# facebookresearch/iSDF

Measured on AMD Instinct MI355X. Metric: train-steps/sec: device-synchronised Trainer.step() on 27k-point ray batches, timed as metrics.start_timing / end_timing bracket it (SURVEY 8d); whole job.  SDF L1 vs GT: sdf_l1_vs_gt, higher is better.
Workload: dtype f16 MFMA operands (compensated forward: hi+lo operands past the cat layer), f32 accumulate; second-order sweeps and dW operands fp16; 1 GPU; replicaCAD.json defaults: 5 keyframes x 200 rays x 27 samples = 27000 points per rank-step, 680x1200 synthetic room depth, 6x256 Softplus MLP + 255-wide icosahedron PE (460033 params), eik+normal loss, bounds=ray, AdamW; stream=680x1200, scaling_mode=weak: every rank draws the full 5 x 200 rays, parallelism=single GPU

## Files before the change

isdf_amd/csrc/capi.hip:

```cpp
#include <cstdio>
#include "isdf_common.h"
#include "chain_params.h"
#include "launchers.h"

using namespace isdf;

namespace isdf { thread_local int g_isdf_last_hip_error = 0; }

extern "C" {

int isdf_abi_version(void) { return ISDF_ABI_VERSION; }

static thread_local int g_isdf_last_collective_error = 0;

const char* isdf_error_string(int code) {
  switch (code) {
    case ISDF_OK: return "ok";
    case ISDF_EINVAL: return "invalid argument";
    case ISDF_EUNSUPPORTED: return "unsupported configuration (the tile kernels take hidden_feature_size <= 512 (zero-padded to 256 / 512), n_freqs = n_embed_funcs+1 in 1..12, any hidden_layers_block up to 7; bounds_method ray|pc)";
    case ISDF_EWORKSPACE: return "workspace too small";
    case ISDF_EHIP: {
      static thread_local char buf[160];
      snprintf(buf, sizeof(buf), "HIP runtime error: %s", g_isdf_last_hip_error ? hipGetErrorString((hipError_t)g_isdf_last_hip_error) : "(no launch status recorded)");
      return buf;
    }
    case ISDF_ECOLLECTIVE: {
      static thread_local char buf[96];
      snprintf(buf, sizeof(buf), "the collective library refused the all-reduce (ncclResult_t %d)", g_isdf_last_collective_error);
      return buf;
    }
  }
  return "unknown error";
}

int isdf_check_net(const isdf_net_cfg* net) {
  NetLayout l; int rc = make_layout(net, &l);
  if (rc) return rc;
  return layout_supported(l) ? ISDF_OK : ISDF_EUNSUPPORTED;
}

int64_t isdf_param_count(const isdf_net_cfg* net) {
  NetLayout l; int rc = make_layout(net, &l);
  return rc ? rc : l.n_params;
}

int64_t isdf_shadow_bytes(const isdf_net_cfg* net) {
  NetLayout l; int rc = make_layout(net, &l);
  return rc ? rc : l.shadowElems * 2;
}

int64_t isdf_workspace_bytes(const isdf_net_cfg* net, int64_t max_points, int32_t train) {
  NetLayout l; int rc = make_layout(net, &l);
  if (rc) return rc;
  if (max_points < 0) return ISDF_EINVAL;
  WorkspaceLayout w; make_workspace(l, max_points, max_points, train != 0, &w);
  return w.totalBytes;
}

int64_t isdf_reduce_floats(const isdf_net_cfg* net, int32_t n_frames) {
  NetLayout l; int rc = make_layout(net, &l);
  if (rc) return rc;
  return reduce_layout(l, n_frames).total;
}

int64_t isdf_reduce_split_floats(const isdf_net_cfg* net) {
  NetLayout l; int rc = make_layout(net, &l);
  if (rc) return rc;
  return l.offW[l.cat];
}

int isdf_pack_weights(const isdf_net_cfg* net, const float* params, void* shadow, void* stream) {
  isdf_clear_stale_hip_error();
  NetLayout l; int rc = make_layout(net, &l);
  if (rc) return rc;
  if (!params || !shadow) return ISDF_EINVAL;
  return launch_pack(l, params, (uint16_t*)shadow, (hipStream_t)stream);
}

int64_t isdf_sample_scan_bytes(int64_t max_rays) { return max_rays < 1 ? ISDF_EINVAL : sample_scan_bytes(max_rays); }

int isdf_sample_rays(const isdf_sample_args* a, const isdf_sample_out* o, void* scan_ws, int64_t scan_ws_bytes,
                     void* stream) {
  isdf_clear_stale_hip_error();
  if (!a || !o || !a->depth_batch || !a->T_WC_batch || !o->n_valid || !o->indices_b ||
      !o->indices_h || !o->indices_w || !o->depth_sample || !o->dirs_C_sample || !o->dirs_W_sample || !o->z_vals ||
      !o->pc)
    return ISDF_EINVAL;
  if (a->n_inline != 0 && (a->n_inline != a->n_frames || a->n_inline > ISDF_MAX_INLINE_FRAMES)) return ISDF_EINVAL;
  for (int f = 0; f < a->n_inline; ++f)
    if (a->frame_idx_inline[f] < 0 || (a->normal_batch && a->normal_idx_inline[f] < 0)) return ISDF_EINVAL;
  if (a->n_inline == 0 && (!a->frame_idx || (a->normal_batch && !a->normal_idx))) return ISDF_EINVAL;
  if (a->n_frames < 1 || a->n_rays < 1 || a->H < 1 || a->W < 1 || a->n_strat < 1 || a->n_surf < 0) return ISDF_EINVAL;
  if ((int64_t)a->n_frames * a->n_rays > 0x7fffffff / 64) return ISDF_EINVAL;
  if (a->rng_mode == 0 && (!a->draw_h || !a->draw_w || !a->draw_u || (a->n_surf > 1 && !a->draw_n))) return ISDF_EINVAL;
  if (!scan_ws || scan_ws_bytes < sample_scan_bytes((int64_t)a->n_frames * a->n_rays)) return ISDF_EWORKSPACE;
  return launch_sample_rays(*a, *o, scan_ws, (hipStream_t)stream);
}

int isdf_sdf_eval(const isdf_net_cfg* net, const float* params, const void* shadow, const float* pts,
                  int64_t n_points, const float* noise, float* sdf, float* sdf_grad, void* workspace,
                  int64_t workspace_bytes, void* stream) {
  isdf_clear_stale_hip_error();
  NetLayout l; int rc = make_layout(net, &l);
  if (rc) return rc;
  if (!layout_supported(l)) return ISDF_EUNSUPPORTED;
  if (!params || !shadow || !pts || !sdf || n_points < 0) return ISDF_EINVAL;
  if (n_points == 0) return ISDF_OK;
  ChainParams p = {};
  p.lay = l; p.params = params; p.shadow = (const uint16_t*)shadow; p.pts = pts; p.noise = noise;
  p.n_points_host = n_points; p.pts_capacity = n_points; p.S = 1; p.sdf = sdf; p.sdf_grad = sdf_grad;
  const int mode = sdf_grad ? 1 : 0;
  WorkspaceLayout w; make_workspace(l, n_points, 0, false, &w);
  if (mode == 1) {
    if (!workspace || workspace_bytes < w.totalBytes) return ISDF_EWORKSPACE;
    p.spill = (uint16_t*)((char*)workspace + w.offSpill); p.sp = w.sp;
  }
  chain_debug_from_env(p.dbg, workspace && workspace_bytes >= 4096 ? (char*)workspace + workspace_bytes - 4096 : nullptr);
  return launch_chain(p, mode, w.nTiles, (hipStream_t)stream);
}

static bool optim_args_ok(const isdf_optim_args* opt, int32_t n_frames) {
  if (!opt || !opt->params || !opt->exp_avg || !opt->exp_avg_sq || !opt->shadow || opt->step < 1) return false;
  if ((opt->loss_approx == nullptr) != (opt->frame_avg == nullptr)) return false;
  if (opt->frame_avg_inline_n != 0 && (opt->frame_avg_inline_n != n_frames || opt->frame_avg_inline_n > ISDF_MAX_INLINE_FRAMES))
    return false;
  for (int f = 0; f < opt->frame_avg_inline_n; ++f)
    if (opt->frame_avg_index_inline[f] < 0) return false;
  return true;
}

static AdamwHyper tail_optim(TailParams& t, const isdf_optim_args& opt) {
  t.params = opt.params; t.m = opt.exp_avg; t.v = opt.exp_avg_sq; t.shadow = (uint16_t*)opt.shadow;
  t.grad_scale = opt.grad_scale;
  FinalizeArgs& f = t.fin;
  f.la_out = opt.loss_approx; f.fa_out = opt.frame_avg; f.fa_index = opt.frame_avg_index;
  f.fa_inline_n = opt.frame_avg_inline_n;
  for (int k = 0; k < opt.frame_avg_inline_n; ++k) f.fa_inline[k] = opt.frame_avg_index_inline[k];
  return AdamwHyper{opt.lr, opt.beta1, opt.beta2, opt.eps, opt.weight_decay, opt.step};
}

static int train_step_impl(const isdf_net_cfg* net, const isdf_loss_cfg* loss, const float* params, const void* shadow,
                           const isdf_step_args* a, const isdf_step_out* o, void* workspace, int64_t workspace_bytes,
                           void* stream, const isdf_optim_args* opt) {
  isdf_clear_stale_hip_error();
  NetLayout l; int rc = make_layout(net, &l);
  if (rc) return rc;
  if (!layout_supported(l)) return ISDF_EUNSUPPORTED;
  if (!loss || !params || !shadow || !a || !o || !workspace || !o->reduce_buf) return ISDF_EINVAL;
  if (!a->pc || !a->z_vals || !a->depth_sample || !a->dirs_C_sample || !a->dirs_W_sample || !a->indices_b ||
      !a->indices_h || !a->indices_w || !a->n_valid)
    return ISDF_EINVAL;
  if (a->max_rays < 1 || a->S < 1 || a->n_frames < 1 || a->H < 8 || a->W < 8) return ISDF_EINVAL;
  if (a->H % 8 != 0 || a->W % 8 != 0 || a->H >= 65536 || a->W >= 65536) return ISDF_EINVAL;
  if (loss->bounds_method != 0 && loss->bounds_method != 1) return ISDF_EUNSUPPORTED;
  if (loss->bounds_method == 1 && (!a->pc_bounds || !a->pc_grad_vec)) return ISDF_EINVAL;
  if (loss->loss_type != 0 && loss->loss_type != 1) return ISDF_EINVAL;
  if (loss->grad_weight != 0.f && !a->norm_sample) return ISDF_EINVAL;
  const int64_t maxPts = (int64_t)a->max_rays * a->S;
  if (maxPts > 0x7fffffff) return ISDF_EINVAL;
  if (a->extra_floats < 0 || a->extra_floats > 1016 || (a->extra_floats > 0 && (a->extra_slot < 0 || a->extra_slot >= a->extra_floats)))
    return ISDF_EINVAL;
  WorkspaceLayout w; make_workspace(l, maxPts, a->max_rays, true, &w);
  if (workspace_bytes < w.totalBytes) return ISDF_EWORKSPACE;
  hipStream_t st = (hipStream_t)stream;
  char* ws = (char*)workspace;
  float* wgLoss = (float*)(ws + w.offWgLoss);
  float* dwPart = (float*)(ws + w.offDwPart);
  float* vecPart = (float*)(ws + w.offVecPart);
  float* totLoss = (float*)(ws + w.offTotLoss);

  ChainParams p = {};
  p.lay = l; p.loss = *loss; p.params = params; p.shadow = (const uint16_t*)shadow;
  p.pts = a->pc; p.pts_capacity = maxPts; p.noise = a->noise; p.n_valid = a->n_valid; p.S = a->S;
  p.noise_std = a->noise_std; p.noise_seed = a->noise_seed; p.noise_off = a->noise_offset;
  p.z_vals = a->z_vals; p.depth = a->depth_sample; p.dirsC = a->dirs_C_sample; p.dirsW = a->dirs_W_sample;
  p.normals = a->norm_sample; p.pc_bounds = a->pc_bounds; p.pc_grad_vec = a->pc_grad_vec;
  p.sdf = o->sdf; p.sdf_grad = o->sdf_grad; p.tot_loss_mat = o->tot_loss_mat;
  p.tot_ws = totLoss; p.wg_loss = wgLoss; p.vec_part = vecPart; p.vecStride = w.vecStride;
  p.spill = (uint16_t*)(ws + w.offSpill); p.sp = w.sp;
  p.pe_aux = (float*)(ws + w.offPeAux);
  chain_debug_from_env(p.dbg, ws + w.totalBytes - 4096);
  hipEvent_t* ev = (hipEvent_t*)o->prof_events;
  if (ev && hipEventRecord(ev[0], st) != hipSuccess) return ISDF_EHIP;
  rc = launch_chain(p, 2, w.nTiles, st);
  if (rc) return rc;
  if (ev && hipEventRecord(ev[1], st) != hipSuccess) return ISDF_EHIP;

  DwParams d = {};
  d.lay = l; d.sp = w.sp; d.spill = p.spill; d.pe_aux = p.pe_aux; d.n_valid = a->n_valid; d.S = a->S; d.cap_tiles = (int32_t)w.nTiles;
  d.dwPart = dwPart;
  rc = launch_dw(d, st);
  if (rc) return rc;
  if (ev && hipEventRecord(ev[2], st) != hipSuccess) return ISDF_EHIP;
  const ReduceLayout r = reduce_layout(l, a->n_frames);
  TailParams t = {};
  t.lay = l; t.dwPart = dwPart; t.vecPart = vecPart; t.vecStride = w.vecStride; t.grad = o->reduce_buf;
  FinalizeArgs& f = t.fin;
  f.wg_loss = wgLoss; f.maxTiles = w.nTiles; f.n_valid = a->n_valid; f.S = a->S; f.tot_ws = totLoss;
  f.ib = a->indices_b; f.ih = a->indices_h; f.iw = a->indices_w; f.n_frames = a->n_frames; f.H = a->H; f.W = a->W;
  f.loss_sums = o->reduce_buf + r.lossSums; f.block_loss = o->reduce_buf + r.blockLoss; f.block_cnt = o->reduce_buf + r.blockCnt;
  f.mailbox = o->host_mailbox; f.extra = o->reduce_buf + r.extra;
  f.n_extra = a->extra_floats; f.extra_slot = a->extra_slot; f.extra_value = a->extra_value;
  if (opt) {
    const AdamwHyper hyper = tail_optim(t, *opt);
    rc = launch_step_tail(0, t, &hyper, 0, st);
    if (rc) return rc;
  }
  const int parts = opt ? 0 : o->split_event ? 2 : 1;
  for (int part = 1; part <= parts; ++part) {
    rc = launch_step_tail(1, t, nullptr, parts == 1 ? 0 : part, st);
    if (rc) return rc;
    if (parts == 2 && part == 1 && hipEventRecord((hipEvent_t)o->split_event, st) != hipSuccess) return ISDF_EHIP;
  }
  if (ev && hipEventRecord(ev[3], st) != hipSuccess) return ISDF_EHIP;
  return ISDF_OK;
}

int isdf_train_step(const isdf_net_cfg* net, const isdf_loss_cfg* loss, const float* params,
                    const void* shadow, const isdf_step_args* a, const isdf_step_out* o,
                    void* workspace, int64_t workspace_bytes, void* stream) {
  return train_step_impl(net, loss, params, shadow, a, o, workspace, workspace_bytes, stream, nullptr);
}

int isdf_train_step_adamw(const isdf_net_cfg* net, const isdf_loss_cfg* loss, const isdf_step_args* a,
                          const isdf_step_out* o, const isdf_optim_args* opt, void* workspace,
                          int64_t workspace_bytes, void* stream) {
  if (!a || !optim_args_ok(opt, a->n_frames)) return ISDF_EINVAL;
  if (o && o->split_event) return ISDF_EINVAL;
  return train_step_impl(net, loss, opt->params, opt->shadow, a, o, workspace, workspace_bytes, stream, opt);
}

int isdf_train_step_finish(const isdf_net_cfg* net, const isdf_optim_args* opt, const float* reduce_buf, int32_t n_frames,
                           int32_t extra_floats, float* host_mailbox, void* stream) {
  isdf_clear_stale_hip_error();
  NetLayout l; int rc = make_layout(net, &l);
  if (rc) return rc;
  if (!layout_supported(l)) return ISDF_EUNSUPPORTED;
  if (!optim_args_ok(opt, n_frames) || !reduce_buf) return ISDF_EINVAL;
  if (opt->loss_approx && n_frames < 1) return ISDF_EINVAL;
  if (extra_floats < 0 || extra_floats > 1016 || n_frames < 0) return ISDF_EINVAL;
  if (extra_floats > 0 && !host_mailbox) return ISDF_EINVAL;
  const ReduceLayout r = reduce_layout(l, n_frames);
  float* msg = const_cast<float*>(reduce_buf);
  TailParams t = {};
  t.lay = l; t.grad = msg; t.count_ptr = reduce_buf + r.lossSums + ISDF_LS_COUNT;
  const AdamwHyper hyper = tail_optim(t, *opt);
  FinalizeArgs& f = t.fin;
  f.n_frames = opt->loss_approx ? n_frames : 0;
  f.loss_sums = msg + r.lossSums; f.block_loss = msg + r.blockLoss; f.block_cnt = msg + r.blockCnt;
  f.extra = msg + r.extra; f.n_extra = extra_floats; f.mailbox = host_mailbox;
  return launch_adamw_pack(t, hyper, (hipStream_t)stream);
}

int isdf_allreduce_sum_f32(isdf_nccl_allreduce_fn nccl_all_reduce, void* comm, float* buf, int64_t count, void* stream) {
  if (!nccl_all_reduce || !comm || !buf || count < 1) return ISDF_EINVAL;
  constexpr int kNcclFloat32 = 7, kNcclSum = 0;
  const int rc = nccl_all_reduce(buf, buf, (size_t)count, kNcclFloat32, kNcclSum, comm, stream);
  if (rc != 0) { g_isdf_last_collective_error = rc; return ISDF_ECOLLECTIVE; }
  return ISDF_OK;
}

int isdf_bounds_pc(const int32_t* n_valid, int32_t max_rays, int32_t S, const float* pc, const float* z_vals,
                   const float* depth_sample, const float* surf_pts, int64_t n_surf, float* bounds, float* grad_vec,
                   void* stream) {
  isdf_clear_stale_hip_error();
  if (!n_valid || !pc || !z_vals || !depth_sample || !bounds || !grad_vec || max_rays < 1 || S < 1) return ISDF_EINVAL;
  if (surf_pts && n_surf < 1) return ISDF_EINVAL;
  return launch_bounds_pc(n_valid, max_rays, S, pc, z_vals, depth_sample, surf_pts, n_surf, bounds, grad_vec,
                          (hipStream_t)stream);
}

int isdf_frame_avg(const float* reduce_buf, int64_t n_params, int32_t n_frames, float* loss_approx,
                   float* frame_avg_loss, const int32_t* frame_avg_index, void* stream) {
  isdf_clear_stale_hip_error();
  if (!reduce_buf || !loss_approx || !frame_avg_loss || n_frames < 1 || n_params < 0) return ISDF_EINVAL;
  const ReduceLayout r = reduce_layout(n_params, n_frames);
  return launch_frame_avg(reduce_buf + r.blockLoss, reduce_buf + r.blockCnt, n_frames, loss_approx, frame_avg_loss, frame_avg_index,
                          (hipStream_t)stream);
}

int isdf_estimate_normals(const float* depth, int32_t H, int32_t W, float fx, float fy, float cx, float cy,
                          float* normals, void* stream) {
  isdf_clear_stale_hip_error();
  if (!depth || !normals || H < 1 || W < 1 || fx == 0.f || fy == 0.f) return ISDF_EINVAL;
  return launch_normals(depth, H, W, fx, fy, cx, cy, normals, (hipStream_t)stream);
}

int isdf_render_depth(const int32_t* n_valid, int64_t n_rays_host, int64_t max_rays, int32_t S, const float* z_vals,
                      const float* sdf, const float* depth_sample, float kf_dist_th, float* view_depth,
                      int32_t* below_count, void* stream) {
  isdf_clear_stale_hip_error();
  if (!z_vals || !sdf || !view_depth || S < 1 || max_rays < 1) return ISDF_EINVAL;
  if (!n_valid && (n_rays_host < 0 || n_rays_host > max_rays)) return ISDF_EINVAL;
  return launch_render_depth(n_valid, n_rays_host, max_rays, S, z_vals, sdf, depth_sample, kf_dist_th, view_depth,
                             below_count, (hipStream_t)stream);
}

int isdf_adamw(const isdf_net_cfg* net, float* params, float* exp_avg, float* exp_avg_sq, const float* grad_sum,
               const float* count_ptr, float grad_scale, float lr, float beta1, float beta2, float eps,
               float weight_decay, int32_t step, void* shadow, void* stream) {
  isdf_clear_stale_hip_error();
  NetLayout l; int rc = make_layout(net, &l);
  if (rc) return rc;
  if (!params || !exp_avg || !exp_avg_sq || !grad_sum || step < 1) return ISDF_EINVAL;
  const AdamwHyper hyper = {lr, beta1, beta2, eps, weight_decay, step};
  if (shadow && layout_supported(l)) {
    TailParams t = {};
    t.lay = l; t.grad = const_cast<float*>(grad_sum); t.count_ptr = count_ptr; t.grad_scale = grad_scale;
    t.params = params; t.m = exp_avg; t.v = exp_avg_sq; t.shadow = (uint16_t*)shadow;
    return launch_adamw_pack(t, hyper, (hipStream_t)stream);
  }
  rc = launch_adamw(params, exp_avg, exp_avg_sq, grad_sum, count_ptr, grad_scale, hyper, l.n_params, (hipStream_t)stream);
  if (rc || !shadow) return rc;
  return launch_pack(l, params, (uint16_t*)shadow, (hipStream_t)stream);
}

static bool mesh_dims_ok(int32_t D0, int32_t D1, int32_t D2) {
  return D0 >= 2 && D1 >= 2 && D2 >= 2 && (int64_t)D0 * D1 * D2 <= 0x7fffffff;
}

int64_t isdf_mesh_ws_bytes(int32_t D0, int32_t D1, int32_t D2) {
  if (!mesh_dims_ok(D0, D1, D2)) return ISDF_EINVAL;
  return mesh_ws_layout((int64_t)D0 * D1 * D2, nullptr, nullptr, nullptr, nullptr);
}

int isdf_marching_cubes(const isdf_mc_args* a, int64_t* counts, float* verts, float* normals, int64_t max_verts,
                        int32_t* faces, int64_t max_faces, void* workspace, int64_t workspace_bytes, void* stream) {
  isdf_clear_stale_hip_error();
  if (!a || !a->volume || !counts || !mesh_dims_ok(a->D0, a->D1, a->D2) || max_verts < 0 || max_faces < 0) return ISDF_EINVAL;
  if ((max_verts > 0 && !verts) || (max_faces > 0 && !faces)) return ISDF_EINVAL;
  if (!workspace || workspace_bytes < isdf_mesh_ws_bytes(a->D0, a->D1, a->D2)) return ISDF_EWORKSPACE;
  float N[9];
  if (a->has_transform) {
    const float* m = a->index_to_world;
    auto M = [m](int r, int c) { return (double)m[4 * r + c]; };
    double cof[9];
    for (int r = 0; r < 3; ++r)
      for (int c = 0; c < 3; ++c) {
        const int r1 = (r + 1) % 3, r2 = (r + 2) % 3, c1 = (c + 1) % 3, c2 = (c + 2) % 3;
        cof[3 * r + c] = M(r1, c1) * M(r2, c2) - M(r1, c2) * M(r2, c1);
      }
    const double det = M(0, 0) * cof[0] + M(0, 1) * cof[1] + M(0, 2) * cof[2];
    if (!(det != 0.0) || !__builtin_isfinite(det)) return ISDF_EINVAL;
    for (int q = 0; q < 9; ++q) N[q] = (float)(cof[q] / det);
  }
  return launch_marching_cubes(a->volume, a->D0, a->D1, a->D2, a->level, a->has_transform ? a->index_to_world : nullptr,
                               a->has_transform ? N : nullptr, counts, verts, normals, max_verts, faces, max_faces, workspace,
                               (hipStream_t)stream);
}

int isdf_mc_tables(int32_t* edge_corners_host, int8_t* tri_table_host) {
  mc_tables_host(edge_corners_host, tri_table_host);
  return ISDF_OK;
}

struct RenderWs { int64_t z, pc, sdf, depth, npts, nsdf, ngrad, fwd, fwdBytes, total; };

static int64_t align256(int64_t x) { return (x + 255) & ~(int64_t)255; }

static int render_ws_layout(const isdf_net_cfg* net, int32_t B, int32_t H, int32_t W, int32_t S, RenderWs* w) {
  if (B < 0 || H < 1 || W < 1 || S < 1) return ISDF_EINVAL;
  NetLayout l; int rc = make_layout(net, &l);
  if (rc) return rc;
  if (!layout_supported(l)) return ISDF_EUNSUPPORTED;
  const int64_t rays = (int64_t)B * H * W, pts = rays * S;
  if ((int64_t)H * W > 0x7fffffff || pts > ((int64_t)1 << 40)) return ISDF_EINVAL;
  WorkspaceLayout fw; make_workspace(l, rays > 0 ? rays : 1, 0, false, &fw);
  int64_t o = 0;
  w->z = o; o = align256(o + 4 * pts);
  w->pc = o; o = align256(o + 12 * pts);
  w->sdf = o; o = align256(o + 4 * pts);
  w->depth = o; o = align256(o + 4 * rays);
  w->npts = o; o = align256(o + 12 * rays);
  w->nsdf = o; o = align256(o + 4 * rays);
  w->ngrad = o; o = align256(o + 12 * rays);
  w->fwd = o; w->fwdBytes = fw.totalBytes; o = align256(o + fw.totalBytes);
  w->total = o;
  return ISDF_OK;
}

int64_t isdf_render_ws_bytes(const isdf_net_cfg* net, int32_t n_views, int32_t H, int32_t W, int32_t n_samples) {
  if (!net) return ISDF_EINVAL;
  RenderWs w; int rc = render_ws_layout(net, n_views, H, W, n_samples, &w);
  return rc ? rc : w.total;
}

int isdf_render_views(const isdf_net_cfg* net, const float* params, const void* shadow, const isdf_render_args* a,
                      float* depth_out, float* normals_out, void* workspace, int64_t workspace_bytes, void* stream) {
  isdf_clear_stale_hip_error();
  if (!net || !a || !params || !shadow || (!depth_out && !normals_out)) return ISDF_EINVAL;
  const bool given = a->depth_in != nullptr;
  const int S = given ? 1 : a->n_samples;
  RenderWs w; int rc = render_ws_layout(net, a->n_views, a->H, a->W, S, &w);
  if (rc) return rc;
  if (a->n_views == 0) return ISDF_OK;
  if (!a->T_WC || !a->dirs_C || (given && !normals_out)) return ISDF_EINVAL;
  if (!given) {
    if (a->range_mode == ISDF_RANGE_SCALAR) {
      if (!(a->bin_length >= 0.f)) return ISDF_EINVAL;
    } else if (a->range_mode == ISDF_RANGE_DEPTH || a->range_mode == ISDF_RANGE_UPSAMPLE) {
      if (!a->src_depth || a->src_H < 1 || a->src_W < 1) return ISDF_EINVAL;
    } else {
      return ISDF_EINVAL;
    }
    if ((a->rng_mode != 0 && a->rng_mode != 1) || (a->rng_mode == 0 && !a->draw_u)) return ISDF_EINVAL;
  }
  if (!workspace || workspace_bytes < w.total) return ISDF_EWORKSPACE;
  hipStream_t st = (hipStream_t)stream;
  char* ws = (char*)workspace;
  const int64_t R = (int64_t)a->H * a->W, rays = (int64_t)a->n_views * R;
  const float* depth = a->depth_in;
  if (!given) {
    float* z = (float*)(ws + w.z);
    float* pc = (float*)(ws + w.pc);
    float* sdf = (float*)(ws + w.sdf);
    float* dst = depth_out ? depth_out : (float*)(ws + w.depth);
    if ((rc = launch_render_samples(*a, z, pc, st))) return rc;
    if ((rc = isdf_sdf_eval(net, params, shadow, pc, rays * S, nullptr, sdf, nullptr, nullptr, 0, stream))) return rc;
    if ((rc = launch_render_depth(nullptr, rays, rays, S, z, sdf, nullptr, 0.f, dst, nullptr, st))) return rc;
    depth = dst;
  }
  if (!normals_out) return ISDF_OK;
  float* npts = (float*)(ws + w.npts);
  float* ngrad = (float*)(ws + w.ngrad);
  if ((rc = launch_normal_points(a->T_WC, a->dirs_C, R, rays, depth, npts, st))) return rc;
  if ((rc = isdf_sdf_eval(net, params, shadow, npts, rays, nullptr, (float*)(ws + w.nsdf), ngrad, ws + w.fwd, w.fwdBytes,
                          stream)))
    return rc;
  return launch_normal_finish(a->T_WC, R, rays, ngrad, normals_out, st);
}

static bool gt_volume_ok(const isdf_gt_volume* vol) {
  if (vol->nx < 2 || vol->ny < 2 || vol->nz < 2 || (int64_t)vol->nx * vol->ny * vol->nz > 0x7fffffff) return false;
  for (int k = 0; k < 3; ++k)
    if (!(vol->spacing[k] > 0.f) || !__builtin_isfinite(vol->spacing[k]) || !__builtin_isfinite(vol->origin[k])) return false;
  return true;
}

int isdf_sdf_metrics(const isdf_gt_volume* vol, const float* pts, const float* sdf, int64_t n, int32_t exclude_zero_gt,
                     float oob_fill, double* record, float* gt_out, uint8_t* valid_out, void* workspace,
                     int64_t workspace_bytes, void* stream) {
  isdf_clear_stale_hip_error();
  if (!vol || !record || n < 0 || (n > 0 && (!pts || !sdf))) return ISDF_EINVAL;
  if (!gt_volume_ok(vol)) return ISDF_EINVAL;
  if (n > 0 && !vol->values) return ISDF_EINVAL;
  if (!workspace || workspace_bytes < ISDF_SDF_METRICS_WS_BYTES) return ISDF_EWORKSPACE;
  return launch_sdf_metrics(*vol, pts, sdf, n, exclude_zero_gt != 0, oob_fill, record, gt_out, valid_out, (double*)workspace,
                            (hipStream_t)stream);
}

int isdf_region_metrics(const isdf_region_args* a, double* records, void* workspace, int64_t workspace_bytes, void* stream) {
  isdf_clear_stale_hip_error();
  if (!a || !records || a->n < 0 || a->n > ((int64_t)1 << 40)) return ISDF_EINVAL;
  if ((a->vol != nullptr) == (a->gt_in != nullptr)) return ISDF_EINVAL;
  if (a->grad_sets && (!a->sdf_grad || a->gt_in)) return ISDF_EINVAL;
  if (!(a->delta > 0.0) || !__builtin_isfinite(a->delta)) return ISDF_EINVAL;
  if (a->vol) {
    if (!gt_volume_ok(a->vol)) return ISDF_EINVAL;
    for (int k = 0; k < 3; ++k)
      if (!(a->spacing[k] > 0.0) || !__builtin_isfinite(a->spacing[k]) || !__builtin_isfinite(a->origin[k])) return ISDF_EINVAL;
    if (a->n > 0 && !a->vol->values) return ISDF_EINVAL;
  }
  if (a->n > 0 && (!a->pts || !a->sdf)) return ISDF_EINVAL;
  if (!workspace || workspace_bytes < ISDF_REGION_METRICS_WS_BYTES) return ISDF_EWORKSPACE;
  return launch_region_metrics(*a, records, (double*)workspace, (hipStream_t)stream);
}

int isdf_nn_distance(const float* query, int64_t n, const float* target, int64_t m, float* dist, int32_t* index,
                     double* dist_sum, void* workspace, int64_t workspace_bytes, void* stream) {
  isdf_clear_stale_hip_error();
  if (!dist_sum || n < 0 || n > ((int64_t)1 << 40) || (n > 0 && (!query || !target || m < 1 || m > 0xfffffffe))) return ISDF_EINVAL;
  if (!workspace || workspace_bytes < ISDF_NN_WS_BYTES(n)) return ISDF_EWORKSPACE;
  unsigned long long* keys = (unsigned long long*)workspace;
  return launch_nn_distance(query, n, target, m, dist, index, dist_sum, keys, (double*)(keys + n), (hipStream_t)stream);
}

int isdf_slice_images(const float* pts, const float* sdf, int64_t n, const isdf_colormap* cmap, const isdf_gt_volume* vol,
                      float oob_fill, float chomp_eps, uint8_t* pred_rgb, float* gt_out, uint8_t* gt_rgb, float* pred_cost,
                      float* gt_cost, void* stream) {
  isdf_clear_stale_hip_error();
  const bool pred = pred_rgb || pred_cost, gt = gt_out || gt_rgb || gt_cost;
  if (n < 0 || n > ((int64_t)1 << 40) || (!pred && !gt)) return ISDF_EINVAL;
  if (gt && !vol) return ISDF_EINVAL;
  if ((pred_rgb || gt_rgb) && !cmap) return ISDF_EINVAL;
  if ((pred_cost || gt_cost) && !(chomp_eps > 0.f && __builtin_isfinite(chomp_eps))) return ISDF_EINVAL;
  if (cmap && (cmap->n_colors < 1 || cmap->n_colors > ISDF_COLORMAP_MAX_COLORS || !(cmap->range > 0.f) ||
               !__builtin_isfinite(cmap->range) || !__builtin_isfinite(cmap->vmin)))
    return ISDF_EINVAL;
  if (vol && !gt_volume_ok(vol)) return ISDF_EINVAL;
  if (n == 0) return ISDF_OK;
  if ((pred && !sdf) || (gt && (!pts || !vol->values)) || (cmap && (pred_rgb || gt_rgb) && !cmap->lut)) return ISDF_EINVAL;
  return launch_slice_images((pred_rgb || gt_rgb) ? cmap : nullptr, gt ? vol : nullptr, pts, pred ? sdf : nullptr, n, oob_fill,
                             chomp_eps, pred_rgb, gt_out, gt_rgb, pred_cost, gt_cost, (hipStream_t)stream);
}

int isdf_plane_points(const float* origin, const float* du, const float* dv, int32_t H, int32_t W, float* pts_out,
                      void* stream) {
  isdf_clear_stale_hip_error();
  if (!origin || !du || !dv || H < 0 || W < 0 || (int64_t)H * W > 0x7fffffff) return ISDF_EINVAL;
  if ((int64_t)H * W == 0) return ISDF_OK;
  if (!pts_out) return ISDF_EINVAL;
  return launch_plane_points(origin, du, dv, H, W, pts_out, (hipStream_t)stream);
// ... 221 lines not shown
```

isdf_amd/csrc/chain_params.h:

```cpp
#pragma once
#include "isdf_common.h"
#include "chain_debug.h"

namespace isdf {

struct ChainParams {
  NetLayout lay;
  isdf_loss_cfg loss;
  const float* params;
  const uint16_t* shadow;
  const float* pts;
  const float* noise;
  float noise_std; uint64_t noise_seed, noise_off;
  const int32_t* n_valid;
  int64_t n_points_host;
  int64_t pts_capacity;
  int32_t S;
  const float* z_vals; const float* depth; const float* dirsC; const float* dirsW; const float* normals;
  const float* pc_bounds; const float* pc_grad_vec;
  float* sdf; float* sdf_grad; float* tot_loss_mat;
  float* tot_ws;
  float* wg_loss;
  float* vec_part;
  int32_t vecStride;
  uint16_t* spill; SpillLayout sp;
  float* pe_aux;
  int32_t n_cu;
  ChainDebug dbg;
};

struct DwParams {
  NetLayout lay;
  SpillLayout sp;
  const uint16_t* spill;
  const float* pe_aux;
  const int32_t* n_valid; int64_t n_points_host; int32_t S;
  int32_t cap_tiles;
  float* dwPart;
};

struct AdamwHyper { float lr, b1, b2, eps, wd; int step; };
struct AdamwCoef { float lr, b1, b2, eps, wd, bc1, bc2_sqrt; };
struct FinalizeArgs {
  const float* wg_loss; int64_t maxTiles; const int32_t* n_valid; int S; const float* tot_ws;
  const int64_t *ib, *ih, *iw; int n_frames, H, W;
  float *loss_sums, *block_loss, *block_cnt;
  float *la_out, *fa_out; const int32_t* fa_index;
  int fa_inline_n; int32_t fa_inline[8];
  float* mailbox; float* extra; int n_extra, extra_slot; float extra_value;
};
static_assert(ISDF_MAX_INLINE_FRAMES == 8, "FinalizeArgs::fa_inline holds isdf_optim_args.frame_avg_index_inline");
struct TailParams {
  NetLayout lay;
  const float* dwPart; const float* vecPart; int32_t vecStride;
  float* grad;
  float *params, *m, *v; uint16_t* shadow;
  AdamwCoef c; float grad_scale;
  const float* count_ptr;
  FinalizeArgs fin;
  int nW, nV;
  int wBlock0;
};

}
```

isdf_amd/csrc/optim.hip:

```cpp
#include "isdf_common.h"
#include "launchers.h"
#include "chain_params.h"

namespace isdf {

__device__ __forceinline__ float adamw_update(float* __restrict__ p, float* __restrict__ m, float* __restrict__ v,
                                              int64_t i, float gsum, float gs, const AdamwCoef& c) {
#pragma clang fp contract(off)
  const float gi = gsum * gs;
  float pi = p[i] * (1.f - c.lr * c.wd);
  const float m0 = m[i], v0 = v[i];
  const float mi = c.b1 * m0 + (1.f - c.b1) * gi;
  const float vi = c.b2 * v0 + (1.f - c.b2) * gi * gi;
  const float denom = sqrtf(vi) / c.bc2_sqrt + c.eps;
  pi -= (c.lr / c.bc1) * (mi / denom);
  p[i] = pi;
  m[i] = mi; v[i] = vi;
  return pi;
}
__global__ void adamw_kernel(float* __restrict__ p, float* __restrict__ m, float* __restrict__ v,
                             const float* __restrict__ g, const float* __restrict__ count_ptr,
                             float grad_scale, AdamwCoef c, int64_t n) {
  const int64_t i = (int64_t)blockIdx.x * blockDim.x + threadIdx.x;
  if (i >= n) return;
  float gs = grad_scale;
  if (count_ptr) { if (*count_ptr == 0.f) return; gs /= *count_ptr; }
  adamw_update(p, m, v, i, g[i], gs, c);
}

__device__ __forceinline__ float fwd_src(const NetLayout& L, const float* P, int li, int row, int k) {
  const int HD = L.HD, H = L.H;
  if (row >= H) return 0.f;
  if (li == 0) return k < L.E ? P[L.offW[0] + (int64_t)row * L.K[0] + k] : 0.f;
  if (li == L.cat) {
    if (k < HD) return k < H ? P[L.offW[li] + (int64_t)row * L.K[li] + k] : 0.f;
    const int e = k - HD;
    return e < L.E ? P[L.offW[li] + (int64_t)row * L.K[li] + H + e] : 0.f;
  }
  return k < H ? P[L.offW[li] + (int64_t)row * L.K[li] + k] : 0.f;
}
__device__ __forceinline__ float bwd_src(const NetLayout& L, const float* P, int li, int row, int k) {
  return (row < L.H && k < L.H) ? P[L.offW[li] + (int64_t)k * L.K[li] + row] : 0.f;
}
__device__ __forceinline__ float g_src(const NetLayout& L, const float* P, int row, int k) {
  if (row >= L.E) return 0.f;
  if (k < L.HD) return k < L.H ? P[L.offW[0] + (int64_t)k * L.K[0] + row] : 0.f;
  return k - L.HD < L.H ? P[L.offW[L.cat] + (int64_t)(k - L.HD) * L.K[L.cat] + L.H + row] : 0.f;
}

__global__ void pack_kernel(NetLayout L, const float* __restrict__ P, uint16_t* __restrict__ shadow) {
  const int64_t gid = (int64_t)blockIdx.x * blockDim.x + threadIdx.x;
  const int64_t perFwd = L.fwdSetElems / 8, perBwd = L.bwdSetElems / 8;
  if (gid >= perFwd + perBwd) return;
  const bool isFwd = gid < perFwd;
  const int64_t e0 = (isFwd ? gid : gid - perFwd) * 8;
  float v[8];
  if (isFwd) {
    int li = 0;
    for (int k = 1; k < L.L; ++k) if (e0 >= L.fwdMat[k]) li = k;
    const int Kp = li == 0 ? L.EP : (li == L.cat ? L.HD + L.EP : L.HD);
    int64_t r = (e0 - L.fwdMat[li]) / 8;
    const int lane = (int)(r & 63); r >>= 6;
    const int ks = (int)(r % (Kp / 16)); const int rb = (int)(r / (Kp / 16));
    const int row = rb * 32 + (lane & 31), k0 = ks * 16 + 8 * (lane >> 5);
#pragma unroll
    for (int t = 0; t < 8; ++t) v[t] = fwd_src(L, P, li, row, k0 + t);
  } else {
    const bool isG = e0 >= L.bwdG;
    int li = 1;
    if (!isG) for (int k = 2; k < L.L; ++k) if (e0 >= L.bwdMat[k]) li = k;
    const int Kp = isG ? 2 * L.HD : L.HD;
    int64_t r = (e0 - (isG ? L.bwdG : L.bwdMat[li])) / 8;
    const int lane = (int)(r & 63); r >>= 6;
    const int ks = (int)(r % (Kp / 16)); const int rb = (int)(r / (Kp / 16));
    const int row = rb * 32 + (lane & 31), k0 = ks * 16 + 8 * (lane >> 5);
#pragma unroll
    for (int t = 0; t < 8; ++t) v[t] = isG ? g_src(L, P, row, k0 + t) : bwd_src(L, P, li, row, k0 + t);
  }
  const uint2 a16 = pack4<true>(v[0], v[1], v[2], v[3]), b16 = pack4<true>(v[4], v[5], v[6], v[7]);
  const uint2 abf = pack4<false>(v[0], v[1], v[2], v[3]), bbf = pack4<false>(v[4], v[5], v[6], v[7]);
  const uint4 hA = L.fwd_f16 ? make_uint4(a16.x, a16.y, b16.x, b16.y) : make_uint4(abf.x, abf.y, bbf.x, bbf.y);
  const uint4 hB = make_uint4(abf.x, abf.y, bbf.x, bbf.y);
  *(uint4*)(shadow + (isFwd ? L.setFwdA : L.setBwdA) + e0) = hA;
  if (!L.bwd_f16) *(uint4*)(shadow + (isFwd ? L.setFwdB : L.setBwdB) + e0) = hB;
  if (L.fwd_x2 && isFwd && (L.fwd_x2_all || e0 >= L.fwdMat[L.cat])) {
    float r[8];
#pragma unroll
    for (int t = 0; t < 8; ++t) r[t] = f16_residual(v[t]);
    const uint2 al = pack4<true>(r[0], r[1], r[2], r[3]), bl = pack4<true>(r[4], r[5], r[6], r[7]);
    *(uint4*)(shadow + L.setFwdLo + e0) = make_uint4(al.x, al.y, bl.x, bl.y);
  }
}

constexpr int FIN_CAP = 12288;
struct FinalizeLds { float sh[16][8]; unsigned long long binS[64]; float binC[64]; int range[2]; int cnt[16][2]; uint32_t keys[FIN_CAP]; };

__device__ __forceinline__ void finalize_block(int block, const FinalizeArgs& a, FinalizeLds& lds) {
  const float* __restrict__ wg_loss = a.wg_loss; const int64_t maxTiles = a.maxTiles; const int S = a.S;
  const float* __restrict__ tot_ws = a.tot_ws;
  const int64_t* __restrict__ ib = a.ib; const int64_t* __restrict__ ih = a.ih; const int64_t* __restrict__ iw = a.iw;
  const int H = a.H, W = a.W;
  float* __restrict__ loss_sums = a.loss_sums; float* __restrict__ block_loss = a.block_loss;
  float* __restrict__ block_cnt = a.block_cnt;
  auto& sh = lds.sh; auto& binS = lds.binS; auto& binC = lds.binC; auto& range = lds.range; auto& keys = lds.keys;
  const int tid = threadIdx.x, lane = tid & 63, wv = tid >> 6;
  const int64_t R = *a.n_valid;
  const int64_t P = R * S;
  if (block == 0) {
    const int64_t nTiles = (P + TILE_PTS - 1) / TILE_PTS;
    float acc[5] = {0.f, 0.f, 0.f, 0.f, 0.f};
    for (int64_t t = tid; t < nTiles && t < maxTiles; t += 1024)
#pragma unroll
      for (int k = 0; k < 5; ++k) acc[k] += wg_loss[t * 8 + k];
#pragma unroll
    for (int k = 0; k < 5; ++k) {
      float v = acc[k];
#pragma unroll
      for (int m = 32; m >= 1; m >>= 1) v += __shfl_xor(v, m, 64);
      if (lane == 0) sh[wv][k] = v;
    }
    __syncthreads();
    if (tid < 8) {
      float v = 0.f;
      if (tid < 5) for (int k = 0; k < 16; ++k) v += sh[k][tid];
      loss_sums[tid] = v;
      if (a.mailbox) a.mailbox[tid] = v;
    }
    if (tid < a.n_extra) a.extra[tid] = tid == a.extra_slot ? a.extra_value : 0.f;
    return;
  }
  const int f = block - 1;
  {
    int c0 = 0, c1 = 0;
    for (int64_t r = tid; r < R; r += 1024) { const int64_t b = ib[r]; c0 += b < f; c1 += b <= f; }
#pragma unroll
    for (int m = 32; m >= 1; m >>= 1) { c0 += __shfl_xor(c0, m, 64); c1 += __shfl_xor(c1, m, 64); }
    if (lane == 0) { lds.cnt[wv][0] = c0; lds.cnt[wv][1] = c1; }
  }
  if (tid < 64) { binS[tid] = 0ull; binC[tid] = 0.f; }
  __syncthreads();
  if (tid < 2) {
    int c = 0;
    for (int k = 0; k < 16; ++k) c += lds.cnt[k][tid];
    range[tid] = c;
  }
  __syncthreads();
  const int lo = range[0], n = range[1] - range[0];
  const bool staged = n <= FIN_CAP;
  if (staged) for (int r = tid; r < n; r += 1024) keys[r] = ((uint32_t)ih[lo + r] << 16) | (uint32_t)iw[lo + r];
  __syncthreads();
  const int hb = H / 8, wb = W / 8;
  for (int r = tid; r < n; r += 1024) {
    const uint32_t h = (uint32_t)ih[lo + r], w = (uint32_t)iw[lo + r];
    const uint32_t key = (h << 16) | w;
    bool dup = false;
    if (staged) { for (int q = r + 1; q < n; ++q) dup |= keys[q] == key; }
    else { for (int q = r + 1; q < n; ++q) dup |= ((((uint32_t)ih[lo + q]) << 16) | (uint32_t)iw[lo + q]) == key; }
    if (dup) continue;
    float s = 0.f;
    const float* tp = tot_ws + (int64_t)(lo + r) * S;
    for (int k = 0; k < S; ++k) s += tp[k];
    const int bin = (int)((h / hb) * 8 + (w / wb));
    atomicAdd(&binS[bin], (unsigned long long)(long long)llrint((double)s * 4294967296.0));
    atomicAdd(&binC[bin], 1.f);
  }
  __syncthreads();
  if (tid < 64) {
    const float bs = (float)((double)(long long)binS[tid] * (1.0 / 4294967296.0));
    block_loss[f * 64 + tid] = bs; block_cnt[f * 64 + tid] = binC[tid];
    if (a.la_out) {
      float c = binC[tid];
      c = c == 0.f ? 1.f : c;
      float v = bs / c;
      a.la_out[f * 64 + tid] = v;
#pragma unroll
      for (int m = 32; m >= 1; m >>= 1) v += __shfl_xor(v, m, 64);
      if (tid == 0) a.fa_out[a.fa_inline_n ? a.fa_inline[f] : (a.fa_index ? a.fa_index[f] : f)] = v / 64.f;
    }
  }
}

__device__ __forceinline__ void shadow_put(const NetLayout& L, uint16_t* sh, bool fwdSet, int64_t elem, float val,
                                           bool withResidual = false) {
  const uint32_t h = pack4<true>(val, 0.f, 0.f, 0.f).x & 0xffffu, b = pack4<false>(val, 0.f, 0.f, 0.f).x & 0xffffu;
  sh[(fwdSet ? L.setFwdA : L.setBwdA) + elem] = (uint16_t)(L.fwd_f16 ? h : b);
  if (!L.bwd_f16) sh[(fwdSet ? L.setFwdB : L.setBwdB) + elem] = (uint16_t)b;
  if (withResidual) sh[L.setFwdLo + elem] = (uint16_t)(pack4<true>(f16_residual(val), 0.f, 0.f, 0.f).x & 0xffffu);
}
__device__ __forceinline__ int64_t packed_elem(int row, int k, int Kp) {
  return ((((int64_t)(row >> 5) * (Kp >> 4) + (k >> 4)) * 64 + (row & 31) + 32 * ((k & 15) >> 3)) << 3) + (k & 7);
}

__device__ __forceinline__ void frame_avg_block(int f, int t, const float* __restrict__ block_loss,
                                                const float* __restrict__ block_cnt, float* __restrict__ loss_approx,
                                                float* __restrict__ frame_avg, const int32_t* __restrict__ fa_index,
                                                int dst_inline = -1) {
  if (t >= 64) return;
  float c = block_cnt[f * 64 + t];
  c = c == 0.f ? 1.f : c;
  float v = block_loss[f * 64 + t] / c;
  loss_approx[f * 64 + t] = v;
#pragma unroll
  for (int m = 32; m >= 1; m >>= 1) v += __shfl_xor(v, m, 64);
  if (t == 0) frame_avg[dst_inline >= 0 ? dst_inline : (fa_index ? fa_index[f] : f)] = v / 64.f;
}

template <int PHASE>
__global__ __launch_bounds__(1024) void step_tail_kernel(const TailParams p) {
  __shared__ FinalizeLds lds;
  const NetLayout& L = p.lay;
  const int HD = L.HD;
  const int b = blockIdx.x;
  if (b >= p.nW + p.nV) {
    if (PHASE != 2) finalize_block(b - p.nW - p.nV, p.fin, lds);
    else if (b - p.nW - p.nV < p.fin.n_frames)
      frame_avg_block(b - p.nW - p.nV, threadIdx.x, p.fin.block_loss, p.fin.block_cnt, p.fin.la_out, p.fin.fa_out, p.fin.fa_index,
                      p.fin.fa_inline_n ? p.fin.fa_inline[b - p.nW - p.nV] : -1);
    else if ((int)threadIdx.x < 8 + p.fin.n_extra)
      p.fin.mailbox[threadIdx.x] = threadIdx.x < 8 ? p.fin.loss_sums[threadIdx.x] : p.fin.extra[threadIdx.x - 8];
    return;
  }
  const int64_t P = PHASE == 2 ? 0 : (int64_t)(*p.fin.n_valid) * p.fin.S;
  float gs = p.grad_scale;
  if (PHASE == 0) gs /= (float)P;
  if (PHASE == 2 && p.count_ptr) gs /= *p.count_ptr;
  const bool emptyBatch = (PHASE == 0 && P == 0) || (PHASE == 2 && p.count_ptr && *p.count_ptr == 0.f);
  if (b < p.nW) {
    const int64_t idx = (int64_t)(b + p.wBlock0) * 1024 + threadIdx.x;
    constexpr int64_t perUnit = (int64_t)DW_BLK * DW_BLK;
    const int unit = (int)(idx / perUnit);
    if (unit >= dw_units(L)) return;
    const DwUnit du = dw_unit(L, unit);
    const int rem = (int)(idx - unit * perUnit);
    const int o = du.ob * DW_BLK + rem / DW_BLK;
    const int ip = du.ib * DW_BLK + rem % DW_BLK;
    const int li = du.li;
    if (o >= L.H) return;
    if (li == 0 && ip >= L.E) return;
    if (li == L.cat && ip >= HD && ip - HD >= L.E) return;
    if ((li != 0 && ip < HD && ip >= L.H)) return;
    const int col = (li == L.cat && ip >= HD) ? L.H + (ip - HD) : ip;
    const int64_t pi = L.offW[li] + (int64_t)o * L.K[li] + col;
    float s = 0.f;
    if (PHASE == 2) s = p.grad[pi];
    else {
      const slab_t* src = (const slab_t*)p.dwPart + (int64_t)dw_slab_base(L, unit) * perUnit + rem;
#pragma unroll
      for (int k = 0; k < DW_SPLIT_REG; ++k) s += __builtin_nontemporal_load(src + (int64_t)k * perUnit);
      if (dw_unit_from_emb(L, du)) {
#pragma unroll
        for (int k = DW_SPLIT_REG; k < DW_SPLIT_PE; ++k) s += __builtin_nontemporal_load(src + (int64_t)k * perUnit);
      }
      p.grad[pi] = s;
      if (PHASE == 1) return;
    }
    if (emptyBatch) return;
    const float w = adamw_update(p.params, p.m, p.v, pi, s, gs, p.c);
    const int KpF = li == 0 ? L.EP : (li == L.cat ? HD + L.EP : HD);
    shadow_put(L, p.shadow, true, L.fwdMat[li] + packed_elem(o, ip, KpF), w, L.fwd_x2 && (L.fwd_x2_all || li >= L.cat));
    if (li >= 1 && ip < HD) shadow_put(L, p.shadow, false, L.bwdMat[li] + packed_elem(ip, o, HD), w);
    if (li == 0) shadow_put(L, p.shadow, false, L.bwdG + packed_elem(ip, o, 2 * HD), w);
    else if (li == L.cat && ip >= HD) shadow_put(L, p.shadow, false, L.bwdG + packed_elem(ip - HD, HD + o, 2 * HD), w);
    return;
  }
  float (*sh)[64] = (float (*)[64])lds.keys;
  const int pi = threadIdx.x & 63, g = threadIdx.x >> 6;
  const int v = (b - p.nW) * 64 + pi;
  const int nVec = L.L * HD + HD + 1;
  const int nTiles = (int)((P + TILE_PTS - 1) / TILE_PTS);
  int slotA = 0, slotB = -1, dst = -1;
  if (v < L.L * HD) { slotA = v; if (v % HD < L.H) dst = L.offB[v / HD] + v % HD; }
  else if (v < L.L * HD + HD) { slotA = v; slotB = v + HD; if (v - L.L * HD < L.H) dst = L.offWout + (v - L.L * HD); }
  else if (v < nVec) { slotA = L.L * HD + 2 * HD; dst = L.offBout; }
  if (PHASE == 2) {
    if (g == 0 && dst >= 0 && !emptyBatch) adamw_update(p.params, p.m, p.v, dst, p.grad[dst], gs, p.c);
    return;
  }
  float s = 0.f, s2 = 0.f;
  if (dst >= 0) {
    int t = g;
    for (; t + 112 < nTiles; t += 128) {
      const float* r0 = p.vecPart + (int64_t)t * p.vecStride;
      float a[8], bb[8];
#pragma unroll
      for (int q = 0; q < 8; ++q) a[q] = r0[(int64_t)(16 * q) * p.vecStride + slotA];
      if (slotB >= 0) {
#pragma unroll
        for (int q = 0; q < 8; ++q) bb[q] = r0[(int64_t)(16 * q) * p.vecStride + slotB];
        s2 += ((bb[0] + bb[1]) + (bb[2] + bb[3])) + ((bb[4] + bb[5]) + (bb[6] + bb[7]));
      }
      s += ((a[0] + a[1]) + (a[2] + a[3])) + ((a[4] + a[5]) + (a[6] + a[7]));
    }
    for (; t + 48 < nTiles; t += 64) {
      const float* r0 = p.vecPart + (int64_t)t * p.vecStride;
      const float a0 = r0[slotA], a1 = r0[(int64_t)16 * p.vecStride + slotA],
                  a2 = r0[(int64_t)32 * p.vecStride + slotA], a3 = r0[(int64_t)48 * p.vecStride + slotA];
      s += (a0 + a1) + (a2 + a3);
      if (slotB >= 0) {
        const float b0 = r0[slotB], b1 = r0[(int64_t)16 * p.vecStride + slotB],
                    b2 = r0[(int64_t)32 * p.vecStride + slotB], b3 = r0[(int64_t)48 * p.vecStride + slotB];
        s2 += (b0 + b1) + (b2 + b3);
      }
    }
    for (; t < nTiles; t += 16) {
      const float* row = p.vecPart + (int64_t)t * p.vecStride;
      s += row[slotA];
      if (slotB >= 0) s2 += row[slotB];
    }
    s += s2;
  }
  sh[g][pi] = s;
  __syncthreads();
  if (g == 0 && dst >= 0) {
    float t = 0.f;
#pragma unroll
    for (int k = 0; k < 16; ++k) t += sh[k][pi];
    p.grad[dst] = t;
    if (PHASE == 0 && !emptyBatch) adamw_update(p.params, p.m, p.v, dst, t, gs, p.c);
  }
}

__global__ void frame_avg_kernel(const float* __restrict__ block_loss, const float* __restrict__ block_cnt,
                                 int n_frames, float* __restrict__ loss_approx, float* __restrict__ frame_avg,
                                 const int32_t* __restrict__ fa_index) {
  frame_avg_block(blockIdx.x, threadIdx.x, block_loss, block_cnt, loss_approx, frame_avg, fa_index);
}

__global__ __launch_bounds__(256) void bounds_pc_kernel(const int32_t* __restrict__ n_valid, int S,
                                                        const float* __restrict__ pc, const float* __restrict__ z_vals,
                                                        const float* __restrict__ depth, const float* __restrict__ surf,
                                                        int64_t n_surf, float* __restrict__ bounds,
                                                        float* __restrict__ grad_vec) {
#pragma clang fp contract(off)
  __shared__ float sx[256], sy[256], sz[256];
  const int64_t Rl = *n_valid, P = Rl * S;
  const int64_t R = surf ? n_surf : Rl;
  const int64_t sstride = surf ? 3 : (int64_t)S * 3;
  const float* sp = surf ? surf : pc;
  const int64_t n = (int64_t)blockIdx.x * 256 + threadIdx.x;
  if ((int64_t)blockIdx.x * 256 >= P) return;
  float px = 0.f, py = 0.f, pz = 0.f;
  if (n < P) { px = pc[n * 3]; py = pc[n * 3 + 1]; pz = pc[n * 3 + 2]; }
  float best = INFINITY; int64_t bi = 0;
  for (int64_t r0 = 0; r0 < R; r0 += 256) {
    const int64_t r = r0 + threadIdx.x;
    __syncthreads();
    if (r < R) { sx[threadIdx.x] = sp[r * sstride]; sy[threadIdx.x] = sp[r * sstride + 1]; sz[threadIdx.x] = sp[r * sstride + 2]; }
    __syncthreads();
    const int cnt = (int)((R - r0) < 256 ? (R - r0) : 256);
    for (int k = 0; k < cnt; ++k) {
      const float dx = px - sx[k], dy = py - sy[k], dz = pz - sz[k];
      const float d2 = (dx * dx + dy * dy) + dz * dz;
      if (d2 < best) { best = d2; bi = r0 + k; }
    }
  }
  if (n >= P) return;
  const int64_t ray = n / S;
  const float dist = sqrtf(best);
  const bool behind = z_vals[n] > depth[ray];
  bounds[n] = behind ? -dist : dist;
  float gx = px - sp[bi * sstride], gy = py - sp[bi * sstride + 1], gz = pz - sp[bi * sstride + 2];
  const float nn = sqrtf(gx * gx + gy * gy + gz * gz);
  gx /= nn; gy /= nn; gz /= nn;
  if (behind) { gx = -gx; gy = -gy; gz = -gz; }
  grad_vec[n * 3] = gx; grad_vec[n * 3 + 1] = gy; grad_vec[n * 3 + 2] = gz;
}

static AdamwCoef adamw_coef(const AdamwHyper& h) {
  const float b1 = h.b1, b2 = h.b2; const int step = h.step;
  return AdamwCoef{h.lr, b1, b2, h.eps, h.wd, 1.f - powf(b1, (float)step), sqrtf(1.f - powf(b2, (float)step))};
}
static void tail_sections(TailParams& p) {
  const int64_t total = (int64_t)dw_units(p.lay) * DW_BLK * DW_BLK;
  p.nW = (int)((total + 1023) / 1024);
  p.nV = (p.lay.L * p.lay.HD + p.lay.HD + 1 + 63) / 64;
}
int launch_adamw(float* p, float* m, float* v, const float* g, const float* cnt, float gs, const AdamwHyper& hyper, int64_t n,
                 hipStream_t st) {
  const AdamwCoef c = adamw_coef(hyper);
  hipLaunchKernelGGL(adamw_kernel, dim3((unsigned)((n + 255) / 256)), dim3(256), 0, st, p, m, v, g, cnt, gs, c, n);
  return isdf_launch_status();
}
int launch_pack(const NetLayout& L, const float* params, uint16_t* shadow, hipStream_t st) {
  const int64_t groups = (L.fwdSetElems + L.bwdSetElems) / 8;
  hipLaunchKernelGGL(pack_kernel, dim3((unsigned)((groups + 255) / 256)), dim3(256), 0, st, L, params, shadow);
  return isdf_launch_status();
}
int launch_step_tail(int phase, const TailParams& block, const AdamwHyper* hyper, int part, hipStream_t st) {
  if ((phase != 0 && phase != 1) || (phase == 0 && !hyper)) return ISDF_EINVAL;
  TailParams p = block;
  const NetLayout& L = p.lay;
  if (phase == 0) p.c = adamw_coef(*hyper);
  tail_sections(p);
  int tailBlocks = p.nV + 1 + p.fin.n_frames;
  if (part != 0) {
    if (phase != 1) return ISDF_EINVAL;
    int unitsBelow = 0;
    for (int li = 0; li < L.cat; ++li) unitsBelow += (L.HD / DW_BLK) * (dw_kpad(L, li) / DW_BLK);
    const int split = unitsBelow * (DW_BLK * DW_BLK / 1024);
    if (part == 1) { p.wBlock0 = split; p.nW -= split; }
    else { p.nW = split; p.nV = 0; tailBlocks = 0; }
  }
  const dim3 grid((unsigned)(p.nW + tailBlocks));
  if (grid.x == 0) return ISDF_OK;
  if (phase == 0) hipLaunchKernelGGL(step_tail_kernel<0>, grid, dim3(1024), 0, st, p);
  else hipLaunchKernelGGL(step_tail_kernel<1>, grid, dim3(1024), 0, st, p);
  return isdf_launch_status();
}
int launch_adamw_pack(const TailParams& block, const AdamwHyper& hyper, hipStream_t st) {
  TailParams p = block;
  p.c = adamw_coef(hyper);
  tail_sections(p);
  hipLaunchKernelGGL(step_tail_kernel<2>, dim3((unsigned)(p.nW + p.nV + p.fin.n_frames + (p.fin.mailbox ? 1 : 0))), dim3(1024), 0, st, p);
  return isdf_launch_status();
}
int launch_frame_avg(const float* bl, const float* bc, int F, float* la, float* fa, const int32_t* fa_index,
                     hipStream_t st) {
  hipLaunchKernelGGL(frame_avg_kernel, dim3(F), dim3(64), 0, st, bl, bc, F, la, fa, fa_index);
  return isdf_launch_status();
}
int launch_bounds_pc(const int32_t* n_valid, int max_rays, int S, const float* pc, const float* z, const float* depth,
                     const float* surf, int64_t n_surf, float* bounds, float* gv, hipStream_t st) {
  const int64_t maxPts = (int64_t)max_rays * S;
  hipLaunchKernelGGL(bounds_pc_kernel, dim3((unsigned)((maxPts + 255) / 256)), dim3(256), 0, st, n_valid, S, pc, z,
                     depth, surf, n_surf, bounds, gv);
  return isdf_launch_status();
}

}
```

Before: 3912 train-steps/s.

## Restructure per-frame finalize: prefetch indices, ballot counts, split dedup scan across threads

The per-frame loss-binning block now prefetches ray indices with buffer loads before waiting on n_valid, counts frame ranges with wave ballots instead of shuffles, and drops one barrier by having every thread sum the per-wave counts. The quadratic duplicate scan splits each ray across up to 64 threads with unrolled LDS reads, and the per-ray loss samples are loaded early. This targets the latency of the serial finalize tail that runs after the optimizer step. It also pins waves-per-EU on the tail kernel, which may constrain registers for the other phases, and adds a max_rays field to the finalize arguments.

```diff
diff --git a/isdf_amd/csrc/capi.hip b/isdf_amd/csrc/capi.hip
--- a/isdf_amd/csrc/capi.hip
+++ b/isdf_amd/csrc/capi.hip
@@ -198,6 +198,7 @@
   FinalizeArgs& f = t.fin;
   f.wg_loss = wgLoss; f.maxTiles = w.nTiles; f.n_valid = a->n_valid; f.S = a->S; f.tot_ws = totLoss;
   f.ib = a->indices_b; f.ih = a->indices_h; f.iw = a->indices_w; f.n_frames = a->n_frames; f.H = a->H; f.W = a->W;
+  f.max_rays = a->max_rays;
   f.loss_sums = o->reduce_buf + r.lossSums; f.block_loss = o->reduce_buf + r.blockLoss; f.block_cnt = o->reduce_buf + r.blockCnt;
   f.mailbox = o->host_mailbox; f.extra = o->reduce_buf + r.extra;
   f.n_extra = a->extra_floats; f.extra_slot = a->extra_slot; f.extra_value = a->extra_value;
diff --git a/isdf_amd/csrc/chain_params.h b/isdf_amd/csrc/chain_params.h
--- a/isdf_amd/csrc/chain_params.h
+++ b/isdf_amd/csrc/chain_params.h
@@ -44,6 +44,7 @@
 struct FinalizeArgs {
   const float* wg_loss; int64_t maxTiles; const int32_t* n_valid; int S; const float* tot_ws;
   const int64_t *ib, *ih, *iw; int n_frames, H, W;
+  int max_rays;
   float *loss_sums, *block_loss, *block_cnt;
   float *la_out, *fa_out; const int32_t* fa_index;
   int fa_inline_n; int32_t fa_inline[8];
diff --git a/isdf_amd/csrc/optim.hip b/isdf_amd/csrc/optim.hip
--- a/isdf_amd/csrc/optim.hip
+++ b/isdf_amd/csrc/optim.hip
@@ -1,6 +1,7 @@
 #include "isdf_common.h"
 #include "launchers.h"
 #include "chain_params.h"
+#include "chain_dev.h"
 
 namespace isdf {
 
@@ -93,7 +94,10 @@
 }
 
 constexpr int FIN_CAP = 12288;
-struct FinalizeLds { float sh[16][8]; unsigned long long binS[64]; float binC[64]; int range[2]; int cnt[16][2]; uint32_t keys[FIN_CAP]; };
+constexpr int FIN_PRE = 4;
+constexpr int FIN_SUM_UNROLL = 32;
+typedef unsigned int u32x2 __attribute__((ext_vector_type(2)));
+struct FinalizeLds { float sh[16][8]; unsigned long long binS[64]; float binC[64]; int cnt[16][2]; uint32_t keys[FIN_CAP]; };
 
 __device__ __forceinline__ void finalize_block(int block, const FinalizeArgs& a, FinalizeLds& lds) {
   const float* __restrict__ wg_loss = a.wg_loss; const int64_t maxTiles = a.maxTiles; const int S = a.S;
@@ -102,11 +106,10 @@
   const int H = a.H, W = a.W;
   float* __restrict__ loss_sums = a.loss_sums; float* __restrict__ block_loss = a.block_loss;
   float* __restrict__ block_cnt = a.block_cnt;
-  auto& sh = lds.sh; auto& binS = lds.binS; auto& binC = lds.binC; auto& range = lds.range; auto& keys = lds.keys;
+  auto& sh = lds.sh; auto& binS = lds.binS; auto& binC = lds.binC; auto& keys = lds.keys;
   const int tid = threadIdx.x, lane = tid & 63, wv = tid >> 6;
-  const int64_t R = *a.n_valid;
-  const int64_t P = R * S;
   if (block == 0) {
+    const int64_t P = (int64_t)(*a.n_valid) * S;
     const int64_t nTiles = (P + TILE_PTS - 1) / TILE_PTS;
     float acc[5] = {0.f, 0.f, 0.f, 0.f, 0.f};
     for (int64_t t = tid; t < nTiles && t < maxTiles; t += 1024)
@@ -130,39 +133,102 @@
     return;
   }
   const int f = block - 1;
+  const int64_t cap = a.max_rays;
+  const uint32_t idxBytes = (uint32_t)(cap < 1024 * FIN_PRE ? cap : 1024 * FIN_PRE) * 8u;
+  const rsrc_t rb = make_rsrc(ib, idxBytes), rh = make_rsrc(ih, idxBytes), rw = make_rsrc(iw, idxBytes);
+  int64_t pb[FIN_PRE]; uint32_t ph[FIN_PRE], pw[FIN_PRE];
+  uint32_t nvRaw = __builtin_amdgcn_raw_buffer_load_b32(make_rsrc(a.n_valid, 4u), 0, 0, 0);
+#pragma unroll
+  for (int j = 0; j < FIN_PRE; ++j) {
+    const int off = (tid + 1024 * j) * 8;
+    const u32x2 b2 = __builtin_amdgcn_raw_buffer_load_b64(rb, off, 0, 0);
+    pb[j] = (int64_t)(((uint64_t)b2[1] << 32) | b2[0]);
+    ph[j] = __builtin_amdgcn_raw_buffer_load_b32(rh, off, 0, 0);
+    pw[j] = __builtin_amdgcn_raw_buffer_load_b32(rw, off, 0, 0);
+  }
+  asm volatile("" : "+v"(nvRaw) : : "memory");
+  const int64_t R = (int32_t)nvRaw;
   {
     int c0 = 0, c1 = 0;
-    for (int64_t r = tid; r < R; r += 1024) { const int64_t b = ib[r]; c0 += b < f; c1 += b <= f; }
-#pragma unroll
-    for (int m = 32; m >= 1; m >>= 1) { c0 += __shfl_xor(c0, m, 64); c1 += __shfl_xor(c1, m, 64); }
+#pragma unroll
+    for (int j = 0; j < FIN_PRE; ++j) {
+      const int64_t g = tid + 1024 * j;
+      const bool in = g < R && g < cap;
+      c0 += __popcll(__ballot(in && pb[j] < f)); c1 += __popcll(__ballot(in && pb[j] <= f));
+    }
+    for (int64_t g = tid + 1024 * FIN_PRE; g < R && g < cap; g += 1024) {
+      const int64_t b = ib[g];
+      c0 += __popcll(__ballot(b < f)); c1 += __popcll(__ballot(b <= f));
+    }
     if (lane == 0) { lds.cnt[wv][0] = c0; lds.cnt[wv][1] = c1; }
   }
   if (tid < 64) { binS[tid] = 0ull; binC[tid] = 0.f; }
   __syncthreads();
-  if (tid < 2) {
-    int c = 0;
-    for (int k = 0; k < 16; ++k) c += lds.cnt[k][tid];
-    range[tid] = c;
-  }
-  __syncthreads();
-  const int lo = range[0], n = range[1] - range[0];
+  int lo = 0, n = 0;
+#pragma unroll
+  for (int k = 0; k < 16; ++k) { lo += lds.cnt[k][0]; n += lds.cnt[k][1]; }
+  n -= lo;
   const bool staged = n <= FIN_CAP;
-  if (staged) for (int r = tid; r < n; r += 1024) keys[r] = ((uint32_t)ih[lo + r] << 16) | (uint32_t)iw[lo + r];
+  if (staged) {
+#pragma unroll
+    for (int j = 0; j < FIN_PRE; ++j) {
+      const int r = tid + 1024 * j - lo;
+      if (r >= 0 && r < n) keys[r] = (ph[j] << 16) | pw[j];
+    }
+    const int r0 = 1024 * FIN_PRE - lo;
+    for (int r = (r0 > 0 ? r0 : 0) + tid; r < n; r += 1024) keys[r] = ((uint32_t)ih[lo + r] << 16) | (uint32_t)iw[lo + r];
+  }
   __syncthreads();
   const int hb = H / 8, wb = W / 8;
-  for (int r = tid; r < n; r += 1024) {
-    const uint32_t h = (uint32_t)ih[lo + r], w = (uint32_t)iw[lo + r];
-    const uint32_t key = (h << 16) | w;
-    bool dup = false;
-    if (staged) { for (int q = r + 1; q < n; ++q) dup |= keys[q] == key; }
-    else { for (int q = r + 1; q < n; ++q) dup |= ((((uint32_t)ih[lo + q]) << 16) | (uint32_t)iw[lo + q]) == key; }
-    if (dup) continue;
-    float s = 0.f;
-    const float* tp = tot_ws + (int64_t)(lo + r) * S;
-    for (int k = 0; k < S; ++k) s += tp[k];
-    const int bin = (int)((h / hb) * 8 + (w / wb));
+  auto bin_ray = [&](uint32_t key, float s) {
+    const int bin = (int)(((key >> 16) / hb) * 8 + ((key & 0xffffu) / wb));
     atomicAdd(&binS[bin], (unsigned long long)(long long)llrint((double)s * 4294967296.0));
     atomicAdd(&binC[bin], 1.f);
+  };
+  if (!staged) {
+    for (int r = tid; r < n; r += 1024) {
+      const uint32_t key = ((uint32_t)ih[lo + r] << 16) | (uint32_t)iw[lo + r];
+      bool dup = false;
+      for (int q = r + 1; q < n; ++q) dup |= ((((uint32_t)ih[lo + q]) << 16) | (uint32_t)iw[lo + q]) == key;
+      if (dup) continue;
+      float s = 0.f;
+      const float* tp = tot_ws + (int64_t)(lo + r) * S;
+      for (int k = 0; k < S; ++k) s += tp[k];
+      bin_ray(key, s);
+    }
+  } else {
+    int tl = 0;
+    if (n > 0 && n < 1024) { tl = 31 - __clz(1024 / n); tl = tl > 6 ? 6 : tl; }
+    const int T = 1 << tl, part = tid & (T - 1);
+    for (int r = tid >> tl; r < n; r += 1024 >> tl) {
+      const uint32_t key = keys[r];
+      const float* tp = tot_ws + (int64_t)(lo + r) * S;
+      float v[FIN_SUM_UNROLL];
+      if (S <= FIN_SUM_UNROLL && part == 0) {
+#pragma unroll
+        for (int k = 0; k < FIN_SUM_UNROLL; ++k) if (k < S) v[k] = tp[k];
+      }
+      bool dup = false;
+      int q = r + 1 + part;
+      for (; q + 3 * T < n; q += 4 * T) {
+        const uint32_t k0 = keys[q], k1 = keys[q + T], k2 = keys[q + 2 * T], k3 = keys[q + 3 * T];
+        dup |= (k0 == key) | (k1 == key) | (k2 == key) | (k3 == key);
+      }
+      for (; q < n; q += T) dup |= keys[q] == key;
+      if (tl > 0) {
+        const unsigned long long grp = (__ballot(dup) >> (lane & ~(T - 1))) & (tl == 6 ? ~0ull : (1ull << T) - 1ull);
+        dup = grp != 0ull;
+      }
+      if (dup || part != 0) continue;
+      float s = 0.f;
+      if (S <= FIN_SUM_UNROLL) {
+#pragma unroll
+        for (int k = 0; k < FIN_SUM_UNROLL; ++k) if (k < S) s += v[k];
+      } else {
+        for (int k = 0; k < S; ++k) s += tp[k];
+      }
+      bin_ray(key, s);
+    }
   }
   __syncthreads();
   if (tid < 64) {
@@ -206,7 +272,7 @@
 }
 
 template <int PHASE>
-__global__ __launch_bounds__(1024) void step_tail_kernel(const TailParams p) {
+__global__ __attribute__((amdgpu_waves_per_eu(8, 8))) __launch_bounds__(1024) void step_tail_kernel(const TailParams p) {
   __shared__ FinalizeLds lds;
   const NetLayout& L = p.lay;
   const int HD = L.HD;
```

Result: no change. 3950 train-steps/s (median of 6 runs) (+1.0%).
